# aous72/OpenJPH

Measured on AMD Instinct MI355X. Metric: Msamples/s encode+decode, 8K 12-bit 4:4:4; achieved HBM GB/s vs roofline, higher is better.
Workload: dtype f32; 1 GPU; c3_8k_444_12b_irv97; width=7680, height=4320, components=3, bit_depth=12, wavelet=9/7 irreversible, decomps=5, hip_streams=1, sample_container_bits=16, roundtrip_max_abs_err=8

## Files before the change

include/ojphgpu.h:

```cpp
#ifndef OJPHGPU_H
#define OJPHGPU_H
#include <stddef.h>
#include <stdint.h>

#ifdef __cplusplus
extern "C" {
#endif

#define OJPHGPU_OK              0
#define OJPHGPU_E_INVALID      -1
#define OJPHGPU_E_NOMEM        -2
#define OJPHGPU_E_HIP          -3
#define OJPHGPU_E_CODESTREAM   -4
#define OJPHGPU_E_OVERFLOW     -5
#define OJPHGPU_E_BLOCK        -6
#define OJPHGPU_E_AGAIN        -7
#define OJPHGPU_E_UNCOLLECTED  -8
#define OJPHGPU_E_BUDGET       -9
#define OJPHGPU_E_QUALITY      -10

#define OJPHGPU_MAX_SUBSAMPLED_COMPS 16
#define OJPHGPU_MAX_COC_COMPS 16
#define OJPHGPU_MAX_LIFT_STEPS 16
#define OJPHGPU_MAX_ATK 4
// ... 276 lines not shown
typedef struct ojphgpu_decoder ojphgpu_decoder;

int  ojphgpu_encoder_create(const ojphgpu_plan* plan, int device, void* stream, ojphgpu_encoder** out);
void ojphgpu_encoder_destroy(ojphgpu_encoder* enc);
int  ojphgpu_encoder_create_tiles(const ojphgpu_plan* plan, int device, void* stream,
                                  uint32_t tile_first, uint32_t tile_count, ojphgpu_encoder** out);
int  ojphgpu_encoder_finish_tiles(ojphgpu_encoder* enc, uint8_t* h_out, size_t cap, size_t* out_len,
                                  uint32_t* tile_part_len);
int  ojphgpu_encoder_finish_tiles_device(ojphgpu_encoder* enc, uint8_t* d_out, size_t cap, size_t* out_len,
                                         uint32_t* tile_part_len);
int  ojphgpu_encoder_create_batch(const ojphgpu_plan* plan, int device, void* stream,
                                  uint32_t num_frames, ojphgpu_encoder** out);
int  ojphgpu_encoder_finish_frame(ojphgpu_encoder* enc, uint32_t frame, uint8_t* h_out, size_t cap,
                                  size_t* out_len);
int  ojphgpu_encoder_run_device(ojphgpu_encoder* enc, const int32_t* d_image);
int  ojphgpu_encoder_run_device16(ojphgpu_encoder* enc, const uint16_t* d_image);
int  ojphgpu_encoder_run_device8(ojphgpu_encoder* enc, const uint8_t* d_image);
int  ojphgpu_encode16(ojphgpu_encoder* enc, const uint16_t* h_image, uint8_t* h_out, size_t cap, size_t* out_len);
int  ojphgpu_encoder_finish(ojphgpu_encoder* enc, uint8_t* h_out, size_t cap, size_t* out_len);
int  ojphgpu_encode(ojphgpu_encoder* enc, const int32_t* h_image, uint8_t* h_out, size_t cap,
                    size_t* out_len);
int  ojphgpu_encoder_coded_bytes(ojphgpu_encoder* enc, uint64_t* bytes);

int  ojphgpu_decoder_create(const ojphgpu_plan* plan, int device, void* stream, ojphgpu_decoder** out);
int  ojphgpu_decoder_create_tiles(const ojphgpu_plan* plan, int device, void* stream,
                                  uint32_t tile_first, uint32_t tile_count, ojphgpu_decoder** out);
int  ojphgpu_decoder_create_batch(const ojphgpu_plan* const* plans, uint32_t num_frames, int device,
                                  void* stream, ojphgpu_decoder** out);
int  ojphgpu_decoder_upload_frame(ojphgpu_decoder* dec, uint32_t frame, const uint8_t* h_codestream,
                                  size_t len);
// ... 236 lines not shown
```

openjph_amd/capi.py:

```python
import ctypes as C
import os

_HERE = os.path.dirname(os.path.abspath(__file__))
LIB_PATH = os.path.join(_HERE, "libojphgpu.so")

OK, E_INVALID, E_NOMEM, E_HIP, E_CODESTREAM, E_OVERFLOW, E_BLOCK, E_AGAIN, E_UNCOLLECTED, E_BUDGET, E_QUALITY = 0, -1, -2, -3, -4, -5, -6, -7, -8, -9, -10
RATE_GRID, STATS_BINS = 241, 80
VIDEO_V410, VIDEO_Y410, VIDEO_R210, VIDEO_R10K, VIDEO_Y4XX, VIDEO_AYUV, VIDEO_BGRA, VIDEO_RGBA, VIDEO_ARGB = range(0x21, 0x2A)
PROG_ORDERS = {"LRCP": 0, "RLCP": 1, "RPCL": 2, "PCRL": 3, "CPRL": 4}


class Coc(C.Structure):
    _fields_ = [
        ("rank", C.c_uint8), ("reversible", C.c_uint8), ("num_decomps", C.c_uint8),
        ("log_block_w", C.c_uint8), ("log_block_h", C.c_uint8), ("has_precincts", C.c_uint8),
        ("reserved", C.c_uint8 * 2), ("precinct_exps", C.c_uint8 * 36),
    ]


class LiftStep(C.Structure):
    _fields_ = [("a", C.c_int32), ("b", C.c_int32), ("e", C.c_int32), ("A", C.c_float)]


class Atk(C.Structure):
# ... 269 lines not shown
    "ojphgpu_encoder_destroy": (None, [C.c_void_p]),
    "ojphgpu_encoder_run_device": (C.c_int, [C.c_void_p, C.c_void_p]),
    "ojphgpu_encoder_finish": (C.c_int, [C.c_void_p, C.c_void_p, C.c_size_t, C.POINTER(C.c_size_t)]),
    "ojphgpu_encode": (C.c_int, [C.c_void_p, C.c_void_p, C.c_void_p, C.c_size_t, C.POINTER(C.c_size_t)]),
    "ojphgpu_encoder_coded_bytes": (C.c_int, [C.c_void_p, C.POINTER(C.c_uint64)]),
    "ojphgpu_decoder_create": (C.c_int, [C.c_void_p, C.c_int, C.c_void_p, C.POINTER(C.c_void_p)]),
    "ojphgpu_decoder_destroy": (None, [C.c_void_p]),
    "ojphgpu_decoder_upload": (C.c_int, [C.c_void_p, C.c_void_p, C.c_size_t]),
    "ojphgpu_decoder_run_device": (C.c_int, [C.c_void_p, C.c_void_p]),
    "ojphgpu_decoder_failed_blocks": (C.c_int, [C.c_void_p, C.POINTER(C.c_uint32)]),
    "ojphgpu_decoder_fused_retries": (C.c_int, [C.c_void_p, C.POINTER(C.c_uint32)]),
    "ojphgpu_decoder_giveup_epoch": (C.c_int, [C.c_void_p, C.POINTER(C.c_uint32), C.POINTER(C.c_uint32)]),
    "ojphgpu_decode": (C.c_int, [C.c_void_p, C.c_void_p, C.c_size_t, C.c_void_p]),
    "ojphgpu_encoder_ht_timing": (C.c_int, [C.c_void_p, C.POINTER(C.c_float), C.c_uint32, C.POINTER(C.c_uint32), C.POINTER(C.c_uint32)]),
    "ojphgpu_encoder_set_timing": (C.c_int, [C.c_void_p, C.c_int]),
    "ojphgpu_decoder_set_timing": (C.c_int, [C.c_void_p, C.c_int]),
    "ojphgpu_encoder_timing": (C.c_int, [C.c_void_p, C.POINTER(C.c_float)]),
    "ojphgpu_decoder_timing": (C.c_int, [C.c_void_p, C.POINTER(C.c_float)]),
    "ojphgpu_encoder_level_timing": (C.c_int, [C.c_void_p, C.POINTER(C.c_float), C.c_uint32, C.POINTER(C.c_uint32)]),
    "ojphgpu_decoder_level_timing": (C.c_int, [C.c_void_p, C.POINTER(C.c_float), C.c_uint32, C.POINTER(C.c_uint32)]),
    "ojphgpu_enc_pipe_create": (C.c_int, [C.c_void_p, C.c_int, C.c_uint32, C.c_int, C.c_uint32, C.POINTER(C.c_void_p)]),
    "ojphgpu_enc_pipe_destroy": (None, [C.c_void_p]),
    "ojphgpu_enc_pipe_acquire": (C.c_int, [C.c_void_p, C.POINTER(C.c_void_p), C.POINTER(C.c_size_t)]),
    "ojphgpu_enc_pipe_submit": (C.c_int, [C.c_void_p]),
    "ojphgpu_enc_pipe_collect": (C.c_int, [C.c_void_p, C.POINTER(C.c_void_p), C.POINTER(C.c_size_t)]),
    "ojphgpu_enc_pipe_stats": (C.c_int, [C.c_void_p, C.POINTER(C.c_double)]),
    "ojphgpu_dec_pipe_create": (C.c_int, [C.c_void_p, C.c_size_t, C.c_int, C.c_int, C.c_uint32, C.c_int, C.c_uint32,
                                          C.POINTER(C.c_void_p)]),
    "ojphgpu_dec_pipe_destroy": (None, [C.c_void_p]),
    "ojphgpu_dec_pipe_plan": (C.c_int, [C.c_void_p, C.POINTER(C.c_void_p)]),
# ... 149 lines not shown
```

openjph_amd/codec.py:

```python
import ctypes as C
import numpy as np

from . import capi
from .capi import check, Params, DwtDesc, DwtRegion, CbDesc, CbResult, ConvertDesc
from .plan import Plan, make_params, parse_codestream

dwt_desc_dtype = np.dtype(DwtDesc)
dwt_region_dtype = np.dtype(DwtRegion)
cb_desc_dtype = np.dtype(CbDesc)
cb_result_dtype = np.dtype(CbResult)
convert_desc_dtype = np.dtype(ConvertDesc)


def _torch():
    import torch
    if not torch.cuda.is_available():
        raise RuntimeError("openjph_amd: no GPU visible (torch.cuda.is_available() is False); "
                           "the HTJ2K hot path has no CPU fallback")
    return torch


def _stream_ptr(torch, device):
    return C.c_void_p(torch.cuda.current_stream(device).cuda_stream)

# ... 146 lines not shown
        torch = _torch()
        assert d_image.is_cuda and tuple(d_image.shape) == self.shape and d_image.is_contiguous()
        self._frame = d_image if self.max_sse is not None else None
        if d_image.dtype in (torch.int16, torch.uint16):
            check(self._lib.ojphgpu_encoder_run_device16(self._h, C.c_void_p(d_image.data_ptr())), "encoder_run_device16")
            return
        if d_image.dtype in (torch.int8, torch.uint8):
            check(self._lib.ojphgpu_encoder_run_device8(self._h, C.c_void_p(d_image.data_ptr())), "encoder_run_device8")
            return
        assert d_image.dtype == torch.int32
        check(self._lib.ojphgpu_encoder_run_device(self._h, C.c_void_p(d_image.data_ptr())), "encoder_run_device")

    def set_timing(self, per_launch: bool):
        check(self._lib.ojphgpu_encoder_set_timing(self._h, int(per_launch)), "encoder_set_timing")

    def coded_bytes(self):
        n = C.c_uint64()
        check(self._lib.ojphgpu_encoder_coded_bytes(self._h, C.byref(n)), "encoder_coded_bytes")
        return int(n.value)

    def finish(self, frame=0) -> bytes:
        if self.max_bytes:
            budget = self.budgets[frame] if self.budgets and 0 <= frame < self.frames else self.max_bytes
            cap = min(budget, self.plan.frame_elems * 4 + 64 * self.plan.num_blocks + (1 << 20))
        elif self.max_sse is not None:
            cap = self.plan.frame_elems * 3 + 64 * self.plan.num_blocks + (1 << 20)
        else:
            cap = self.coded_bytes() // self.frames * 2 + 64 * self.plan.num_blocks + (1 << 20)
        out = np.empty(cap, np.uint8)
        n = C.c_size_t()
# ... 771 lines not shown
```

openjph_amd/csrc/ojphgpu_codec.cpp:

```cpp
#include <hip/hip_runtime.h>

#include <algorithm>
#include <chrono>
#include <cstdio>
#include <cstdlib>
#include <cstring>
#include <memory>
#include <mutex>
#include <new>
#include <vector>

#include "ht_tables.h"
#include "ojph_plan.h"
#include "ojph_pool.h"

using namespace ojphgpu;

namespace ojphgpu {

int ensure_tables()
{
  static std::mutex mu;
  static bool done[64] = { false };
  int dev = 0;
// ... 4 lines not shown
  static bool built = false;
  if (!built) { build_ht_tables(tables); built = true; }
  if (upload_enc_tables(tables) != 0 || upload_dec_tables(tables) != 0) return -1;
  done[dev] = true;
  return 0;
}

}

#include "ojphgpu_objects.h"

extern "C" void ojphgpu_encoder_destroy(ojphgpu_encoder* e)
{
  if (!e) return;
  (void)hipSetDevice(e->device);
  for (DeviceBuf* b : { &e->arena, &e->image, &e->dwt_descs, &e->img_descs, &e->cb_descs, &e->conv_descs, &e->scratch, &e->out,
                        &e->results, &e->counters, &e->regions }) b->release();
  e->h_out.release(); e->h_res.release();
  if (e->side) (void)hipStreamDestroy(e->side);
  if (e->ev_fork) (void)hipEventDestroy(e->ev_fork);
  if (e->ev_join) (void)hipEventDestroy(e->ev_join);
  e->timer.destroy();
  delete e->quality;
  delete e->rate;
  delete e;
}

extern "C" int ojphgpu_encoder_create(const ojphgpu_plan* plan, int device, void* stream, ojphgpu_encoder** out)
{
  if (!plan) return OJPHGPU_E_INVALID;
  return ojphgpu_encoder_create_tiles(plan, device, stream, 0, (uint32_t)plan->plan.tiles.size(), out);
}

static int encoder_create(const ojphgpu_plan* plan, int device, void* stream, uint32_t tile_first, uint32_t tile_count,
                          uint32_t nframes, ojphgpu_encoder** out, bool blocks_only = false);

extern "C" int ojphgpu_encoder_create_tiles(const ojphgpu_plan* plan, int device, void* stream, uint32_t tile_first,
                                             uint32_t tile_count, ojphgpu_encoder** out)
{
  return no_throw([&] { return encoder_create(plan, device, stream, tile_first, tile_count, 1, out); });
}

extern "C" int ojphgpu_encoder_create_batch(const ojphgpu_plan* plan, int device, void* stream, uint32_t num_frames,
                                             ojphgpu_encoder** out)
{
  if (!plan) return OJPHGPU_E_INVALID;
  return no_throw([&] { return encoder_create(plan, device, stream, 0, (uint32_t)plan->plan.tiles.size(), num_frames, out); });
}

static void encoder_block_layout(ojphgpu_encoder* e, const uint32_t* band_kmax, std::vector<ojphgpu_cb_desc>& bd, uint64_t& scratch_total,
                                 bool* clamped = nullptr)
{
  if (clamped) *clamped = false;
  const Plan& P = *e->P;
  const uint32_t nframes = e->nframes;
// ... 51 lines not shown
        if (clamped) *clamped = true;
        R = 0; break;
      }
      e->h_regions[2 * r] = (uint32_t)total; e->h_regions[2 * r + 1] = (uint32_t)c;
      total += c;
    }
    e->nreg = R;
    if (R) cap = total; else e->h_regions.clear();
    e->counters_bytes = R ? (size_t)R * 128 : 16;
  }
  e->out_cap = (uint32_t)cap;
  scratch_total = scratch_bytes;
}

static int encoder_create(const ojphgpu_plan* plan, int device, void* stream, uint32_t tile_first, uint32_t tile_count,
                          uint32_t nframes, ojphgpu_encoder** out, bool blocks_only)
{
  if (!plan || !out || nframes == 0) return OJPHGPU_E_INVALID;
  *out = nullptr;
  if ((uint64_t)tile_first + tile_count > plan->plan.tiles.size()) return OJPHGPU_E_INVALID;
  if (plan->plan.skip_read || plan->plan.skip_recon) return OJPHGPU_E_INVALID;
  HIPCHK(hipSetDevice(device));
  if (ensure_tables() != 0) return OJPHGPU_E_HIP;
  ojphgpu_encoder* e = new (std::nothrow) ojphgpu_encoder();
  if (!e) return OJPHGPU_E_NOMEM;
  struct Owner { ojphgpu_encoder* p; ~Owner() { if (p) ojphgpu_encoder_destroy(p); } } owner{ e };
  const Plan& P = plan->plan;
  e->handle = plan; e->P = &P; e->device = device; e->stream = (hipStream_t)stream;
  auto bail = [&](int rc) { return rc; };

  e->tiles = TileRange{ tile_first, tile_count };
// ... 14 lines not shown
    auto top = [&](uint32_t id) { const Band& B = P.bands[P.blocks[id].band]; return B.res == P.style(B.comp).L; };
    auto mid = std::stable_partition(e->block_ids.begin(), e->block_ids.end(), top);
    e->n_top = (uint32_t)(mid - e->block_ids.begin());
    {
      static const int share_env = [] { const char* v = getenv("OJPHGPU_ENC_TOP_SHARE"); const int x = v ? atoi(v) : 0; return x < 10 ? 0 : x > 100 ? 100 : x; }();
      double s_top = 0, s_low = 0;
      for (size_t i = 0; i < e->block_ids.size(); ++i) {
        const Block& k = P.blocks[e->block_ids[i]];
        (i < e->n_top ? s_top : s_low) += (double)k.r.w * k.r.h * 1e-6;
      }
      double dwt_us = 0, level_bytes = 8.0 * (s_top + s_low) * 1e6 / 4.0;
      for (uint32_t l = 2; l <= max_recon_decomps(P); ++l, level_bytes /= 4.0) dwt_us += std::max(12.0, level_bytes / 3.0e6);
      const double us_per_ms = 3.8, margin_us = 30.0;
      const double move = (s_top + margin_us / us_per_ms - 1.6 * s_low - dwt_us / us_per_ms) / 2.0;
      int share = share_env;
      if (!share) share = s_top > 0 && move > 0 ? (int)(100.0 * (1.0 - move / s_top)) : 100;
      share = share < 50 ? 50 : share > 100 ? 100 : share;
      e->n_top = (uint32_t)((uint64_t)e->n_top * (uint32_t)share / 100u);
    }
    if (e->n_top == 0 || e->n_top == e->block_ids.size()) e->n_top = 0;
    else {
      int prio_lo = 0, prio_hi = 0;
      (void)hipDeviceGetStreamPriorityRange(&prio_lo, &prio_hi);
      const char* pe = getenv("OJPHGPU_ENC_SIDE_PRIO");
      const int prio = pe && pe[0] == 'l' ? prio_lo : pe && pe[0] == 'h' ? prio_hi : (prio_lo + prio_hi) / 2;
      if (hipStreamCreateWithPriority(&e->side, hipStreamNonBlocking, pe ? prio : 0) != hipSuccess ||
          hipEventCreateWithFlags(&e->ev_fork, hipEventDisableTiming) != hipSuccess ||
          hipEventCreateWithFlags(&e->ev_join, hipEventDisableTiming) != hipSuccess) return bail(OJPHGPU_E_HIP);
    }
  }
  std::vector<ojphgpu_cb_desc> bd;
  uint64_t scratch_bytes = 0;
  encoder_block_layout(e, nullptr, bd, scratch_bytes);
  const uint64_t cap = e->out_cap;

  if ((!blocks_only && (e->arena.alloc(P.arena_elems * 4 * nframes) || e->dwt_descs.alloc(dd.size() * sizeof(dd[0])) ||
                        e->img_descs.alloc(idd.size() * sizeof(dd[0])) || e->conv_descs.alloc(cd.size() * sizeof(cd[0])))) ||
      e->cb_descs.alloc(bd.size() * sizeof(bd[0])) ||
      e->scratch.alloc(scratch_bytes) || e->out.alloc(cap) ||
      e->results.alloc(bd.size() * sizeof(ojphgpu_cb_result)) || e->counters.alloc(e->counters_bytes) ||
      (e->nreg && e->regions.alloc(e->h_regions.size() * 4)))
    return bail(OJPHGPU_E_NOMEM);
  if (e->nreg && hipMemcpy(e->regions.p, e->h_regions.data(), e->h_regions.size() * 4, hipMemcpyHostToDevice) != hipSuccess) return bail(OJPHGPU_E_HIP);
// ... 15 lines not shown
extern "C" int ojphgpu_encoder_run_device16(ojphgpu_encoder* e, const uint16_t* d_image) { return ojphgpu_encoder_run_container(e, d_image, 16); }
extern "C" int ojphgpu_encoder_run_device8(ojphgpu_encoder* e, const uint8_t* d_image) { return ojphgpu_encoder_run_container(e, d_image, 8); }

namespace {
struct BlockCoderRun {
  ojphgpu_encoder* e; uint8_t* out; ojphgpu_cb_result* res; uint32_t* cnt; uint32_t nblocks; Spans* T;
  bool forked = false;
  int launch(hipStream_t st, uint32_t first, uint32_t n, int widths) {
    const int sh = T ? T->begin(SP_HT_ENC, st) : -1;
    int rc = ojphgpu::ht_encode_launch(st, (const ojphgpu_cb_desc*)e->cb_descs.p + first, n, e->arena.p, (uint8_t*)e->scratch.p, out,
                                       e->out_cap, res + first, cnt, cnt + 1, widths, (const uint32_t*)e->regions.p, e->nreg);
    if (rc) return rc;
    if (T) T->end(sh, st);
    return OJPHGPU_OK;
  }
  int clear() { HIPCHK(hipMemsetAsync(cnt, 0, e->counters_bytes, e->stream)); return OJPHGPU_OK; }
  int fork_top() {
    forked = true;
    HIPCHK(hipEventRecord(e->ev_fork, e->stream));
    HIPCHK(hipStreamWaitEvent(e->side, e->ev_fork, 0));
    int rc = launch(e->side, 0, e->n_top, e->widths_top);
    if (rc) return rc;
    HIPCHK(hipEventRecord(e->ev_join, e->side));
    return OJPHGPU_OK;
  }
  int rest_and_join() {
    int rc = e->n_top && !forked ? fork_top() : OJPHGPU_OK;
    if (rc) return rc;
    rc = launch(e->stream, e->n_top, nblocks - e->n_top, e->widths_rest);
    if (rc) return rc;
    if (e->n_top) HIPCHK(hipStreamWaitEvent(e->stream, e->ev_join, 0));
    return OJPHGPU_OK;
  }
};
}

int ojphgpu_encoder_run_container(ojphgpu_encoder* e, const void* d_image, int container)
{
  if (!e || !d_image) return OJPHGPU_E_INVALID;
  const Plan& P = *e->P;
  if (container != 32 && container != 16 && container != 8) return OJPHGPU_E_INVALID;
  if (container != 32) for (const CompGeo& g : P.comps) if (g.bit_depth > (uint32_t)container) return OJPHGPU_E_INVALID;
  hipStream_t s = e->stream;
  Spans& T = e->timer;
  BlockCoderRun coder{ e, (uint8_t*)(e->o_out ? e->o_out : e->out.p),
                       (ojphgpu_cb_result*)(e->o_results ? e->o_results : e->results.p),
                       (uint32_t*)(e->o_counters ? e->o_counters : e->counters.p), (uint32_t)e->block_ids.size() * e->nframes, &T };
  int rc = coder.clear();
  if (rc) return rc;
  T.start(s);
  if (e->need_convert) {
    const int sp = T.begin(SP_CONVERT, s);
    rc = ojphgpu_convert_forward_ex(s, &P.p, (const ojphgpu_convert_desc*)e->conv_descs.p, e->tiles.count * e->nframes,
                                    e->conv_max_w, e->conv_max_h, d_image, e->arena.p, container);
    T.end(sp, s);
  }
  if (rc) return rc;
  const bool budget = e->searches();
  for (size_t i = 0; i < e->batches.size(); ++i) {
    const LevelBatch& b = e->batches[i];
    const int sp = T.begin(SP_DWT, s);
    if (b.img_first >= 0) {
      ojphgpu_params pp = P.p; pp.reversible = b.rev ? 1 : 0; pp.bit_depth = b.img_depth; pp.is_signed = b.img_signed;
      const ojphgpu_dwt_desc* idesc = (const ojphgpu_dwt_desc*)e->img_descs.p + b.img_first;
      rc = b.general ? ojphgpu_dwt_forward_general_image(s, &b.k, &pp, idesc, b.count, b.max_w, b.max_h, d_image, e->arena.p, container)
                     : ojphgpu_dwt_forward_image_ex(s, &pp, idesc, b.count, b.max_w, b.max_h, d_image, e->arena.p, container, b.nc == 3);
    } else if (b.general)
      rc = ojphgpu_dwt_forward_general(s, &b.k, (const ojphgpu_dwt_desc*)e->dwt_descs.p + b.first, b.count, b.max_w, b.max_h, e->arena.p);
    else
      rc = ojphgpu_dwt_forward(s, b.rev ? 1 : 0, (const ojphgpu_dwt_desc*)e->dwt_descs.p + b.first, b.count,
                               b.max_w, b.max_h, e->arena.p);
    if (rc) return rc;
    T.end(sp, s);
    const bool top_done = b.depth == 0 && (i + 1 == e->batches.size() || e->batches[i + 1].depth != 0);
    if (!budget && e->n_top && top_done && (rc = coder.fork_top()) != 0) return rc;
  }
  if (e->quality_on) {
    T.finish(s);
    e->quality->frame = d_image; e->quality->container = container;
    e->rate->searched = false;
    e->ran = true; e->fetched = false;
    return OJPHGPU_OK;
  }
  if (budget) {
    EncoderRate& R = *e->rate;
    HIPCHK(hipMemsetAsync(R.hist.p, 0, R.hist.n, s));
    const int sp = T.begin(SP_STATS, s);
    rc = ojphgpu_band_stats(s, (const ojphgpu_stats_desc*)R.stats_descs.p, R.n_stats, R.stats_max_w, R.stats_max_h, e->arena.p, (uint32_t*)R.hist.p);
    if (rc) return rc;
    T.end(sp, s);
    T.finish(s);
    R.searched = false;
    e->ran = true; e->fetched = false;
    return OJPHGPU_OK;
  }
  if ((rc = coder.rest_and_join()) != 0) return rc;
  T.finish(s);
  e->ran = true; e->fetched = false;
  return OJPHGPU_OK;
}

extern "C" int ojphgpu_encoder_set_timing(ojphgpu_encoder* e, int per_launch)
{
  if (!e) return OJPHGPU_E_INVALID;
  e->timer.detail = per_launch != 0;
  return OJPHGPU_OK;
}

extern "C" int ojphgpu_encoder_coded_bytes(ojphgpu_encoder* e, uint64_t* bytes)
{
  if (!e || !bytes || !e->ran) return OJPHGPU_E_INVALID;
  e->h_cursors.assign(e->counters_bytes / 4, 0);
  HIPCHK(hipMemcpyAsync(e->h_cursors.data(), e->counters.p, e->counters_bytes, hipMemcpyDeviceToHost, e->stream));
  HIPCHK(hipStreamSynchronize(e->stream));
  uint64_t total = e->h_cursors[0];
  for (uint32_t r = 1; r < e->nreg; ++r) total += e->h_cursors[32 * (size_t)r];
  *bytes = total;
  return e->h_cursors[1] ? OJPHGPU_E_OVERFLOW : OJPHGPU_OK;
}

static int encoder_fetch(ojphgpu_encoder* e, uint32_t frame, std::vector<ojphgpu_coded_block>& cb)
{
  if (frame >= e->nframes) return OJPHGPU_E_INVALID;
  const Plan& P = e->searches() ? e->rate->frame_plan[frame]->plan : *e->P;
  if (!e->fetched) {
    int rc = ojphgpu_encoder_coded_bytes(e, &e->nbytes);
// ... 108 lines not shown
    if (lay.alloc(boff + L.blob.size() + 64)) return OJPHGPU_E_NOMEM;
    struct Free { DeviceBuf& b; ~Free() { b.release(); } } fr{ lay };
    if (jbytes) HIPCHK(hipMemcpyAsync(lay.p, L.jobs.data(), jbytes, hipMemcpyHostToDevice, e->stream));
    if (!L.blob.empty()) HIPCHK(hipMemcpyAsync((uint8_t*)lay.p + boff, L.blob.data(), L.blob.size(), hipMemcpyHostToDevice, e->stream));
    rc = assemble_launch(e->stream, (const T2Job*)lay.p, (uint32_t)L.jobs.size(), (const uint8_t*)lay.p + boff,
                         (const uint8_t*)(e->o_out ? e->o_out : e->out.p), d_out);
    if (rc) return rc;
    HIPCHK(hipStreamSynchronize(e->stream));
    return OJPHGPU_OK;
  });
}

static int encoder_restore_descs(ojphgpu_encoder* e)
{
  HIPCHK(hipSetDevice(e->device));
  HIPCHK(hipStreamSynchronize(e->stream));
  const std::vector<ojphgpu_cb_desc>& bd = e->rate->bd;
  if (!bd.empty()) HIPCHK(hipMemcpy(e->cb_descs.p, bd.data(), bd.size() * sizeof(bd[0]), hipMemcpyHostToDevice));
  e->ran = false;
  return OJPHGPU_OK;
}

static bool encoder_may_search(const ojphgpu_encoder* e)
{
  const Plan& P = *e->P;
  return e->tiles.first == 0 && e->tiles.count == P.tiles.size() && !e->o_out && rate_plan_ok(P);
}

static int encoder_rate_setup(ojphgpu_encoder* e);

// ... 51 lines not shown
    const uint32_t nc = R->table.nclasses;
    std::vector<uint32_t> kfine(P.bands.size());
    for (size_t i = 0; i < kfine.size(); ++i) kfine[i] = R->table.quant[(size_t)(OJPHGPU_RATE_GRID - 1) * nc + R->table.band_class[i]].K_max;
    std::vector<ojphgpu_cb_desc>& bd = R->bd;
    uint64_t scratch_bytes = 0;
    {
      const uint32_t out_cap = e->out_cap, nreg = e->nreg; const size_t counters_bytes = e->counters_bytes;
      const std::vector<uint32_t> regions = e->h_regions;
      bool clamped = false;
      encoder_block_layout(e, kfine.data(), bd, scratch_bytes, &clamped);
      if (clamped && nframes > 1) {
        e->out_cap = out_cap; e->nreg = nreg; e->counters_bytes = counters_bytes; e->h_regions = regions;
        return OJPHGPU_E_INVALID;
      }
    }
    HIPCHK(hipStreamSynchronize(e->stream));
    if (e->side) HIPCHK(hipStreamSynchronize(e->side));
    e->scratch.release(); e->out.release(); e->regions.release(); e->counters.release();
    if (e->scratch.alloc(scratch_bytes) || e->out.alloc(e->out_cap) || e->counters.alloc(e->counters_bytes) ||
        (e->nreg && e->regions.alloc(e->h_regions.size() * 4)) ||
        R->stats_descs.alloc(sd.size() * sizeof(sd[0])) || R->hist.alloc(P.bands.size() * OJPHGPU_STATS_BINS * 4 * nframes) ||
        R->block_class.alloc(cls.size() * 4) || R->quant.alloc((size_t)nc * sizeof(BandQuant) * nframes))
      return OJPHGPU_E_NOMEM;
    if (e->nreg) HIPCHK(hipMemcpy(e->regions.p, e->h_regions.data(), e->h_regions.size() * 4, hipMemcpyHostToDevice));
    if (!bd.empty()) HIPCHK(hipMemcpy(e->cb_descs.p, bd.data(), bd.size() * sizeof(bd[0]), hipMemcpyHostToDevice));
    if (!sd.empty()) HIPCHK(hipMemcpy(R->stats_descs.p, sd.data(), sd.size() * sizeof(sd[0]), hipMemcpyHostToDevice));
    if (!cls.empty()) HIPCHK(hipMemcpy(R->block_class.p, cls.data(), cls.size() * 4, hipMemcpyHostToDevice));
    R->h_hist.assign(P.bands.size() * OJPHGPU_STATS_BINS * nframes, 0);
    R->h_quant.assign((size_t)nc * nframes, BandQuant{ 0.0f, 0 });
    e->rate = R; owner.p = nullptr;
// ... 373 lines not shown
}

extern "C" int ojphgpu_encode(ojphgpu_encoder* e, const int32_t* h_image, uint8_t* h_out, size_t cap, size_t* out_len)
{
  return encode_host(e, h_image, 32, h_out, cap, out_len);
}

extern "C" int ojphgpu_encode16(ojphgpu_encoder* e, const uint16_t* h_image, uint8_t* h_out, size_t cap, size_t* out_len)
{
  return encode_host(e, h_image, 16, h_out, cap, out_len);
}

extern "C" int ojphgpu_encoder_timing(ojphgpu_encoder* e, float out[4])
{
  if (!e || !out || !e->ran) return OJPHGPU_E_INVALID;
  if (e->timer.read(SP_CONVERT, &out[0]) || e->timer.read(SP_DWT, &out[1]) || e->timer.read(SP_HT_ENC, &out[2]) ||
      e->timer.read(-1, &out[3])) return OJPHGPU_E_HIP;
  return OJPHGPU_OK;
}

extern "C" int ojphgpu_encoder_ht_timing(ojphgpu_encoder* e, float* out, uint32_t cap, uint32_t* n, uint32_t* n_top)
{
  if (!e || !out || !n || !e->ran) return OJPHGPU_E_INVALID;
  int k = e->timer.read_each(SP_HT_ENC, out, cap);
  if (k < 0) return OJPHGPU_E_HIP;
  *n = (uint32_t)k;
  if (n_top) *n_top = e->n_top;
  return OJPHGPU_OK;
}

extern "C" int ojphgpu_encoder_level_timing(ojphgpu_encoder* e, float* out, uint32_t cap, uint32_t* n)
{
  if (!e || !out || !n || !e->ran) return OJPHGPU_E_INVALID;
  int k = e->timer.read_each(SP_DWT, out, cap);
  if (k < 0) return OJPHGPU_E_HIP;
  *n = (uint32_t)k;
  return OJPHGPU_OK;
}

extern "C" void ojphgpu_decoder_destroy(ojphgpu_decoder* d)
{
  if (!d) return;
  (void)hipSetDevice(d->device);
  for (DeviceBuf* b : { &d->arena, &d->image, &d->dwt_descs, &d->img_descs, &d->cb_descs, &d->conv_descs, &d->data, &d->status, &d->quads, &d->aux,
                       &d->fstate, &d->dwt_regs, &d->img_regs })
    b->release();
  if (d->h_retry) (void)hipHostFree(d->h_retry);
  if (d->h_stage) (void)hipHostFree(d->h_stage);
// ... 887 lines not shown
```

openjph_amd/csrc/ojphgpu_objects.h:

```cpp
#ifndef OJPHGPU_OBJECTS_H
#define OJPHGPU_OBJECTS_H
#include <hip/hip_runtime.h>

#include <algorithm>
#include <cstdint>
#include <cstdlib>
#include <cstring>
#include <map>
#include <vector>

#include "dwt_region.h"
#include "ht_tables.h"
#include "ojph_plan.h"

using namespace ojphgpu;

namespace {

#define HIPCHK(x) do { if ((x) != hipSuccess) return OJPHGPU_E_HIP; } while (0)

struct DeviceBuf {
  void* p = nullptr; size_t n = 0;
  int alloc(size_t bytes) { n = bytes; return hipMalloc(&p, bytes ? bytes : 16) == hipSuccess ? 0 : -1; }
  void release() { if (p) (void)hipFree(p); p = nullptr; }
// ... 317 lines not shown
std::vector<uint32_t> blocks_of_tiles(const Plan& P, TileRange tr)
{
  std::vector<uint32_t> ids;
  for (size_t i = 0; i < P.blocks.size(); ++i) {
    const Band& B = P.bands[P.blocks[i].band];
    if (P.has_region && !P.reg_blocks[i]) continue;
    if (tr.has(B.tile) && B.res <= P.top_read_res(B.comp)) ids.push_back((uint32_t)i);
  }
  return ids;
}

struct Spans {
  struct Span { hipEvent_t a, b; int kind; };
  std::vector<Span> pool;
  size_t used = 0;
  hipEvent_t t0 = nullptr, t1 = nullptr;
  bool ok = false;
  bool detail = true;
  int init() { ok = hipEventCreate(&t0) == hipSuccess && hipEventCreate(&t1) == hipSuccess; return ok ? 0 : -1; }
  void destroy() {
    for (Span& x : pool) { (void)hipEventDestroy(x.a); (void)hipEventDestroy(x.b); }
    if (t0) (void)hipEventDestroy(t0);
    if (t1) (void)hipEventDestroy(t1);
    pool.clear();
  }
  void start(hipStream_t s) { used = 0; if (ok) (void)hipEventRecord(t0, s); }
  void finish(hipStream_t s) { if (ok) (void)hipEventRecord(t1, s); }
  int begin(int kind, hipStream_t s) {
    if (!ok || !detail) return -1;
    if (used == pool.size()) {
      Span x{ nullptr, nullptr, kind };
      if (hipEventCreate(&x.a) != hipSuccess || hipEventCreate(&x.b) != hipSuccess) { ok = false; return -1; }
      pool.push_back(x);
    }
    pool[used].kind = kind;
    (void)hipEventRecord(pool[used].a, s);
    return (int)used++;
  }
  void end(int id, hipStream_t s) { if (ok && id >= 0) (void)hipEventRecord(pool[(size_t)id].b, s); }
  int read(int kind, float* out) {
    if (!ok || hipEventSynchronize(t1) != hipSuccess) return -1;
    if (kind < 0) return hipEventElapsedTime(out, t0, t1) == hipSuccess ? 0 : -1;
    float sum = 0;
    for (size_t i = 0; i < used; ++i)
      if (pool[i].kind == kind) { float ms = 0; if (hipEventElapsedTime(&ms, pool[i].a, pool[i].b) != hipSuccess) return -1; sum += ms; }
    *out = sum;
    return 0;
  }
  int read_each(int kind, float* out, uint32_t cap) {
    if (!ok || hipEventSynchronize(t1) != hipSuccess) return -1;
    int n = 0;
    for (size_t i = 0; i < used; ++i)
      if (pool[i].kind == kind && (uint32_t)n < cap) { if (hipEventElapsedTime(&out[n], pool[i].a, pool[i].b) != hipSuccess) return -1; ++n; }
    return n;
  }
};
enum { SP_CONVERT = 0, SP_DWT = 1, SP_HT_ENC = 2, SP_PREP = 3, SP_STEP1 = 4, SP_STEP2 = 5, SP_REFINE = 6, SP_STATS = 7 };
// ... 48 lines not shown
  std::vector<LevelBatch> batches;
  uint32_t conv_max_w = 0, conv_max_h = 0, out_cap = 0;
  TileRange tiles{ 0, 0 };
  uint32_t nframes = 1;
  bool fetched = false;
  uint64_t nbytes = 0;
  std::vector<uint32_t> block_ids;
  std::vector<ojphgpu_cb_result> h_results;
  HostBuf h_out, h_res;
  Spans timer;
  bool ran = false;
  uint32_t n_top = 0;
  int widths_top = 0, widths_rest = 0;
  hipStream_t side = nullptr;
  hipEvent_t ev_fork = nullptr, ev_join = nullptr;
  void* o_out = nullptr; void* o_results = nullptr; void* o_counters = nullptr;
  uint32_t nreg = 0;
  std::vector<uint32_t> h_regions, h_cursors;
  DeviceBuf regions;
  size_t counters_bytes = 16;
  std::vector<uint64_t> budgets;
  EncoderRate* rate = nullptr;
  bool quality_on = false; uint64_t max_sse = 0;
  uint64_t cap_bytes = 0;
  EncoderQuality* quality = nullptr;
  bool searches() const { return !budgets.empty() || quality_on; }
};
struct RateTrialOut {
  void* out; ojphgpu_cb_result* d_results; uint32_t* d_counters;
  const ojphgpu_cb_result* h_results; uint32_t* d_publish; const uint32_t* h_publish; hipEvent_t done;
};
int64_t ojphgpu_encoder_rate_trial(ojphgpu_encoder* e, Plan& Q, const RateTrialOut& o, uint32_t j);
struct QualityTrialIo {
  const void* frame; int container;
  ojphgpu_requant_desc* h_descs; const void* d_descs;
  const ojphgpu_frame_err* h_err; void* d_err; hipEvent_t done;
};
int ojphgpu_encoder_quality_trial(ojphgpu_encoder* e, const QualityTrialIo& io, uint32_t j, ojphgpu_frame_err* comps);
int ojphgpu_encoder_run_container(ojphgpu_encoder* e, const void* d_image, int container);

inline void ojphgpu_coded_blocks(const Plan& P, const std::vector<uint32_t>& block_ids, const ojphgpu_cb_result* res,
                                 std::vector<ojphgpu_coded_block>& cb)
{
  cb.assign(P.blocks.size(), ojphgpu_coded_block{ 0, 0, 0, 0, 0 });
  for (size_t i = 0; i < block_ids.size(); ++i) {
    const ojphgpu_cb_result& r = res[i];
    ojphgpu_coded_block& c = cb[block_ids[i]];
    c.offset = r.offset; c.len1 = r.length; c.len2 = 0;
    c.missing_msbs = r.length ? P.bands[P.blocks[block_ids[i]].band].K_max - 1 : 0;
    c.num_passes = r.length ? 1 : 0;
  }
}

struct PadCopy { uint64_t src, dst; uint32_t got, total; };
// ... 84 lines not shown
```

openjph_amd/csrc/ojphgpu_pipe.cpp:

```cpp
#include <chrono>
#include <condition_variable>
#include <deque>
#include <mutex>
#include <new>
#include <thread>

#include "ojphgpu_objects.h"
#include "ojph_pool.h"
#include "video_formats.h"

namespace ojphgpu {
int assemble_launch(void* stream, const T2Job* d_jobs, uint32_t njobs, const uint8_t* d_blob, const uint8_t* d_data, uint8_t* d_out);
int copy_to_host_launch(void* stream, void* d_dst, const void* src, size_t bytes);
int publish_words_launch(void* stream, uint32_t* d_dst, const uint32_t* src, uint32_t n);
int gather_runs_launch(void* stream, const void* d_src, size_t src_cap, const void* d_runs, uint32_t nruns, void* d_dst, uint64_t staged_len);
}

namespace {

struct Pinned {
  uint8_t* p = nullptr; uint8_t* d = nullptr; size_t cap = 0;
  int reserve(size_t bytes) {
    if (bytes <= cap) return 0;
    release();
// ... 499 lines not shown
extern "C" int ojphgpu_enc_pipe_create(const ojphgpu_plan* plan, int device, uint32_t depth, int container_bits,
                                        uint32_t host_threads, ojphgpu_enc_pipe** out)
{
  if (!plan || !out || depth < 2 || depth > 16 || (container_bits != 8 && container_bits != 16 && container_bits != 32)) return OJPHGPU_E_INVALID;
  *out = nullptr;
  return no_throw([&]() -> int {
    HIPCHK(hipSetDevice(device));
    ojphgpu_enc_pipe* p = new (std::nothrow) ojphgpu_enc_pipe();
    if (!p) return OJPHGPU_E_NOMEM;
    struct Owner { ojphgpu_enc_pipe* p; ~Owner() { if (p) ojphgpu_enc_pipe_destroy(p); } } owner{ p };
    const Plan& P = plan->plan;
    p->handle = plan; p->P = &P; p->device = device; p->container = container_bits; p->depth = depth;
    if (container_bits != 32) for (const CompGeo& g : P.comps) if (g.bit_depth > (uint32_t)container_bits) return OJPHGPU_E_INVALID;
    for (hipStream_t* s : { &p->s_h2d, &p->s_comp }) HIPCHK(hipStreamCreateWithFlags(s, hipStreamNonBlocking));
    HIPCHK(create_copy_out_stream(&p->s_d2h));
    int rc = ojphgpu_encoder_create(plan, device, p->s_comp, &p->enc);
    if (rc) return rc;
    (void)ojphgpu_encoder_set_timing(p->enc, 0);
    ojphgpu_encoder* e = p->enc;
    const size_t nb = e->block_ids.size();
    p->frame_bytes = (size_t)P.frame_elems * (size_t)(container_bits / 8);
    p->ho.bytes = p->frame_bytes;
    p->res_bytes = nb * sizeof(ojphgpu_cb_result) + 16;
    const size_t cs_guess = std::min<size_t>((size_t)e->out_cap, (size_t)P.frame_elems + (1u << 20));
    p->slots.resize(depth);
    for (EncSlot& s : p->slots) {
      if (s.h_in.reserve(p->frame_bytes + 64) || s.o.h_res.reserve(p->res_bytes + 64) || s.h_cs.reserve(cs_guess)) return OJPHGPU_E_NOMEM;
      if (s.image.alloc(p->frame_bytes + 64) || s.o.out.alloc((size_t)e->out_cap + 64) || s.o.counters.alloc(e->counters_bytes) ||
          s.cs.reserve(cs_guess)) return OJPHGPU_E_NOMEM;
      const size_t lay_guess = nb * sizeof(T2Job) + nb * 8 + (1u << 16);
      if (s.h_lay.reserve(lay_guess)) return OJPHGPU_E_NOMEM;
// ... 945 lines not shown
```

Before: 107,800 Msamples/s.

## Release encoder's HT block coding onto low-priority streams without joining main stream

When the encoder forks the top-level HT block coding onto a side stream, the remaining blocks now go onto a second low-priority stream instead of the main stream. Neither branch is joined back to the main stream; the encoder is marked pending and every later consumer (clear, coded_bytes, timing, restore, destroy) first settles by making the main stream wait on both branch events. This aims to let the tail of HT encoding overlap with subsequent work such as the decode or the next frame. The cost is extra synchronisation bookkeeping and a risk of missed settle points, so the pipe encoder opts out by using a joined-only constructor.

```diff
diff --git a/include/ojphgpu.h b/include/ojphgpu.h
--- a/include/ojphgpu.h
+++ b/include/ojphgpu.h
@@ -314,6 +314,7 @@
 int  ojphgpu_encoder_finish_frame(ojphgpu_encoder* enc, uint32_t frame, uint8_t* h_out, size_t cap,
                                   size_t* out_len);
 int  ojphgpu_encoder_run_device(ojphgpu_encoder* enc, const int32_t* d_image);
+int  ojphgpu_encoder_is_pending(const ojphgpu_encoder* enc, int* pending);
 int  ojphgpu_encoder_run_device16(ojphgpu_encoder* enc, const uint16_t* d_image);
 int  ojphgpu_encoder_run_device8(ojphgpu_encoder* enc, const uint8_t* d_image);
 int  ojphgpu_encode16(ojphgpu_encoder* enc, const uint16_t* h_image, uint8_t* h_out, size_t cap, size_t* out_len);
diff --git a/openjph_amd/capi.py b/openjph_amd/capi.py
--- a/openjph_amd/capi.py
+++ b/openjph_amd/capi.py
@@ -307,6 +307,7 @@
     "ojphgpu_decode": (C.c_int, [C.c_void_p, C.c_void_p, C.c_size_t, C.c_void_p]),
     "ojphgpu_encoder_ht_timing": (C.c_int, [C.c_void_p, C.POINTER(C.c_float), C.c_uint32, C.POINTER(C.c_uint32), C.POINTER(C.c_uint32)]),
     "ojphgpu_encoder_set_timing": (C.c_int, [C.c_void_p, C.c_int]),
+    "ojphgpu_encoder_is_pending": (C.c_int, [C.c_void_p, C.POINTER(C.c_int)]),
     "ojphgpu_decoder_set_timing": (C.c_int, [C.c_void_p, C.c_int]),
     "ojphgpu_encoder_timing": (C.c_int, [C.c_void_p, C.POINTER(C.c_float)]),
     "ojphgpu_decoder_timing": (C.c_int, [C.c_void_p, C.POINTER(C.c_float)]),
diff --git a/openjph_amd/codec.py b/openjph_amd/codec.py
--- a/openjph_amd/codec.py
+++ b/openjph_amd/codec.py
@@ -184,6 +184,11 @@
     def set_timing(self, per_launch: bool):
         check(self._lib.ojphgpu_encoder_set_timing(self._h, int(per_launch)), "encoder_set_timing")
 
+    def pending(self):
+        n = C.c_int()
+        check(self._lib.ojphgpu_encoder_is_pending(self._h, C.byref(n)), "encoder_is_pending")
+        return bool(n.value)
+
     def coded_bytes(self):
         n = C.c_uint64()
         check(self._lib.ojphgpu_encoder_coded_bytes(self._h, C.byref(n)), "encoder_coded_bytes")
diff --git a/openjph_amd/csrc/ojphgpu_codec.cpp b/openjph_amd/csrc/ojphgpu_codec.cpp
--- a/openjph_amd/csrc/ojphgpu_codec.cpp
+++ b/openjph_amd/csrc/ojphgpu_codec.cpp
@@ -42,12 +42,17 @@
 {
   if (!e) return;
   (void)hipSetDevice(e->device);
+  if (e->side) (void)hipStreamSynchronize(e->side);
+  if (e->low) (void)hipStreamSynchronize(e->low);
+  e->pending = false;
   for (DeviceBuf* b : { &e->arena, &e->image, &e->dwt_descs, &e->img_descs, &e->cb_descs, &e->conv_descs, &e->scratch, &e->out,
                         &e->results, &e->counters, &e->regions }) b->release();
   e->h_out.release(); e->h_res.release();
   if (e->side) (void)hipStreamDestroy(e->side);
+  if (e->low) (void)hipStreamDestroy(e->low);
   if (e->ev_fork) (void)hipEventDestroy(e->ev_fork);
   if (e->ev_join) (void)hipEventDestroy(e->ev_join);
+  if (e->ev_low) (void)hipEventDestroy(e->ev_low);
   e->timer.destroy();
   delete e->quality;
   delete e->rate;
@@ -61,12 +66,18 @@
 }
 
 static int encoder_create(const ojphgpu_plan* plan, int device, void* stream, uint32_t tile_first, uint32_t tile_count,
-                          uint32_t nframes, ojphgpu_encoder** out, bool blocks_only = false);
+                          uint32_t nframes, ojphgpu_encoder** out, bool blocks_only = false, bool joined_only = false);
 
 extern "C" int ojphgpu_encoder_create_tiles(const ojphgpu_plan* plan, int device, void* stream, uint32_t tile_first,
                                              uint32_t tile_count, ojphgpu_encoder** out)
 {
   return no_throw([&] { return encoder_create(plan, device, stream, tile_first, tile_count, 1, out); });
+}
+
+int ojphgpu_encoder_create_joined(const ojphgpu_plan* plan, int device, void* stream, ojphgpu_encoder** out)
+{
+  if (!plan) return OJPHGPU_E_INVALID;
+  return no_throw([&] { return encoder_create(plan, device, stream, 0, (uint32_t)plan->plan.tiles.size(), 1, out, false, true); });
 }
 
 extern "C" int ojphgpu_encoder_create_batch(const ojphgpu_plan* plan, int device, void* stream, uint32_t num_frames,
@@ -148,7 +159,7 @@
 }
 
 static int encoder_create(const ojphgpu_plan* plan, int device, void* stream, uint32_t tile_first, uint32_t tile_count,
-                          uint32_t nframes, ojphgpu_encoder** out, bool blocks_only)
+                          uint32_t nframes, ojphgpu_encoder** out, bool blocks_only, bool joined_only)
 {
   if (!plan || !out || nframes == 0) return OJPHGPU_E_INVALID;
   *out = nullptr;
@@ -193,8 +204,7 @@
       const double us_per_ms = 3.8, margin_us = 30.0;
       const double move = (s_top + margin_us / us_per_ms - 1.6 * s_low - dwt_us / us_per_ms) / 2.0;
       int share = share_env;
-      if (!share) share = s_top > 0 && move > 0 ? (int)(100.0 * (1.0 - move / s_top)) : 100;
-      share = share < 50 ? 50 : share > 100 ? 100 : share;
+      if (!share) { share = s_top > 0 && move > 0 ? (int)(100.0 * (1.0 - move / s_top)) : 100; share = share < 50 ? 50 : share > 100 ? 100 : share; }
       e->n_top = (uint32_t)((uint64_t)e->n_top * (uint32_t)share / 100u);
     }
     if (e->n_top == 0 || e->n_top == e->block_ids.size()) e->n_top = 0;
@@ -203,9 +213,15 @@
       (void)hipDeviceGetStreamPriorityRange(&prio_lo, &prio_hi);
       const char* pe = getenv("OJPHGPU_ENC_SIDE_PRIO");
       const int prio = pe && pe[0] == 'l' ? prio_lo : pe && pe[0] == 'h' ? prio_hi : (prio_lo + prio_hi) / 2;
-      if (hipStreamCreateWithPriority(&e->side, hipStreamNonBlocking, pe ? prio : 0) != hipSuccess ||
+      const char* rel = getenv("OJPHGPU_ENC_RELEASE");
+      e->can_release = !blocks_only && !joined_only && !(rel && rel[0] == '0');
+      const int own_prio = pe ? prio : e->can_release ? prio_lo : 0;
+      if (hipStreamCreateWithPriority(&e->side, hipStreamNonBlocking, own_prio) != hipSuccess ||
           hipEventCreateWithFlags(&e->ev_fork, hipEventDisableTiming) != hipSuccess ||
           hipEventCreateWithFlags(&e->ev_join, hipEventDisableTiming) != hipSuccess) return bail(OJPHGPU_E_HIP);
+      if (e->can_release &&
+          (hipStreamCreateWithPriority(&e->low, hipStreamNonBlocking, own_prio) != hipSuccess ||
+           hipEventCreateWithFlags(&e->ev_low, hipEventDisableTiming) != hipSuccess)) return bail(OJPHGPU_E_HIP);
     }
   }
   std::vector<ojphgpu_cb_desc> bd;
@@ -251,16 +267,18 @@
     if (T) T->end(sh, st);
     return OJPHGPU_OK;
   }
-  int clear() { HIPCHK(hipMemsetAsync(cnt, 0, e->counters_bytes, e->stream)); return OJPHGPU_OK; }
-  int fork_top() {
+  int clear() { int rc = encoder_settle(e); if (rc) return rc; HIPCHK(hipMemsetAsync(cnt, 0, e->counters_bytes, e->stream)); return OJPHGPU_OK; }
+  int fork_top(bool release = false) {
     forked = true;
     HIPCHK(hipEventRecord(e->ev_fork, e->stream));
     HIPCHK(hipStreamWaitEvent(e->side, e->ev_fork, 0));
     int rc = launch(e->side, 0, e->n_top, e->widths_top);
     if (rc) return rc;
     HIPCHK(hipEventRecord(e->ev_join, e->side));
+    if (release) { e->pending = true; HIPCHK(hipStreamWaitEvent(e->low, e->ev_fork, 0)); }
     return OJPHGPU_OK;
   }
+  int rest_released() { return launch(e->low, e->n_top, nblocks - e->n_top, e->widths_rest); }
   int rest_and_join() {
     int rc = e->n_top && !forked ? fork_top() : OJPHGPU_OK;
     if (rc) return rc;
@@ -269,6 +287,10 @@
     if (e->n_top) HIPCHK(hipStreamWaitEvent(e->stream, e->ev_join, 0));
     return OJPHGPU_OK;
   }
+};
+struct ReleasedBranch {
+  ojphgpu_encoder* e; bool armed = false;
+  ~ReleasedBranch() { if (armed) (void)hipEventRecord(e->ev_low, e->low); }
 };
 }
 
@@ -285,6 +307,8 @@
                        (uint32_t*)(e->o_counters ? e->o_counters : e->counters.p), (uint32_t)e->block_ids.size() * e->nframes, &T };
   int rc = coder.clear();
   if (rc) return rc;
+  const bool release = encoder_releases(e);
+  ReleasedBranch branch{ e };
   T.start(s);
   if (e->need_convert) {
     const int sp = T.begin(SP_CONVERT, s);
@@ -310,7 +334,10 @@
     if (rc) return rc;
     T.end(sp, s);
     const bool top_done = b.depth == 0 && (i + 1 == e->batches.size() || e->batches[i + 1].depth != 0);
-    if (!budget && e->n_top && top_done && (rc = coder.fork_top()) != 0) return rc;
+    if (!budget && e->n_top && top_done) {
+      if ((rc = coder.fork_top(release)) != 0) return rc;
+      if (release) { s = e->low; branch.armed = true; }
+    }
   }
   if (e->quality_on) {
     T.finish(s);
@@ -331,8 +358,13 @@
     e->ran = true; e->fetched = false;
     return OJPHGPU_OK;
   }
-  if ((rc = coder.rest_and_join()) != 0) return rc;
-  T.finish(s);
+  if (release && coder.forked) {
+    if ((rc = coder.rest_released()) != 0) return rc;
+    T.finish_two(s, e->side);
+  } else {
+    if ((rc = coder.rest_and_join()) != 0) return rc;
+    T.finish(s);
+  }
   e->ran = true; e->fetched = false;
   return OJPHGPU_OK;
 }
@@ -344,9 +376,18 @@
   return OJPHGPU_OK;
 }
 
+extern "C" int ojphgpu_encoder_is_pending(const ojphgpu_encoder* e, int* pending)
+{
+  if (!e || !pending) return OJPHGPU_E_INVALID;
+  *pending = e->pending ? 1 : 0;
+  return OJPHGPU_OK;
+}
+
 extern "C" int ojphgpu_encoder_coded_bytes(ojphgpu_encoder* e, uint64_t* bytes)
 {
   if (!e || !bytes || !e->ran) return OJPHGPU_E_INVALID;
+  int rc = encoder_settle(e);
+  if (rc) return rc;
   e->h_cursors.assign(e->counters_bytes / 4, 0);
   HIPCHK(hipMemcpyAsync(e->h_cursors.data(), e->counters.p, e->counters_bytes, hipMemcpyDeviceToHost, e->stream));
   HIPCHK(hipStreamSynchronize(e->stream));
@@ -485,6 +526,8 @@
 static int encoder_restore_descs(ojphgpu_encoder* e)
 {
   HIPCHK(hipSetDevice(e->device));
+  int rc = encoder_settle(e);
+  if (rc) return rc;
   HIPCHK(hipStreamSynchronize(e->stream));
   const std::vector<ojphgpu_cb_desc>& bd = e->rate->bd;
   if (!bd.empty()) HIPCHK(hipMemcpy(e->cb_descs.p, bd.data(), bd.size() * sizeof(bd[0]), hipMemcpyHostToDevice));
@@ -566,6 +609,7 @@
         return OJPHGPU_E_INVALID;
       }
     }
+    { const int rc = encoder_settle(e); if (rc) return rc; }
     HIPCHK(hipStreamSynchronize(e->stream));
     if (e->side) HIPCHK(hipStreamSynchronize(e->side));
     e->scratch.release(); e->out.release(); e->regions.release(); e->counters.release();
@@ -969,6 +1013,7 @@
 extern "C" int ojphgpu_encoder_timing(ojphgpu_encoder* e, float out[4])
 {
   if (!e || !out || !e->ran) return OJPHGPU_E_INVALID;
+  if (encoder_settle(e)) return OJPHGPU_E_HIP;
   if (e->timer.read(SP_CONVERT, &out[0]) || e->timer.read(SP_DWT, &out[1]) || e->timer.read(SP_HT_ENC, &out[2]) ||
       e->timer.read(-1, &out[3])) return OJPHGPU_E_HIP;
   return OJPHGPU_OK;
@@ -977,6 +1022,7 @@
 extern "C" int ojphgpu_encoder_ht_timing(ojphgpu_encoder* e, float* out, uint32_t cap, uint32_t* n, uint32_t* n_top)
 {
   if (!e || !out || !n || !e->ran) return OJPHGPU_E_INVALID;
+  if (encoder_settle(e)) return OJPHGPU_E_HIP;
   int k = e->timer.read_each(SP_HT_ENC, out, cap);
   if (k < 0) return OJPHGPU_E_HIP;
   *n = (uint32_t)k;
@@ -987,6 +1033,7 @@
 extern "C" int ojphgpu_encoder_level_timing(ojphgpu_encoder* e, float* out, uint32_t cap, uint32_t* n)
 {
   if (!e || !out || !n || !e->ran) return OJPHGPU_E_INVALID;
+  if (encoder_settle(e)) return OJPHGPU_E_HIP;
   int k = e->timer.read_each(SP_DWT, out, cap);
   if (k < 0) return OJPHGPU_E_HIP;
   *n = (uint32_t)k;
diff --git a/openjph_amd/csrc/ojphgpu_objects.h b/openjph_amd/csrc/ojphgpu_objects.h
--- a/openjph_amd/csrc/ojphgpu_objects.h
+++ b/openjph_amd/csrc/ojphgpu_objects.h
@@ -355,18 +355,21 @@
   struct Span { hipEvent_t a, b; int kind; };
   std::vector<Span> pool;
   size_t used = 0;
-  hipEvent_t t0 = nullptr, t1 = nullptr;
+  hipEvent_t t0 = nullptr, t1 = nullptr, t2 = nullptr;
   bool ok = false;
   bool detail = true;
-  int init() { ok = hipEventCreate(&t0) == hipSuccess && hipEventCreate(&t1) == hipSuccess; return ok ? 0 : -1; }
+  bool two = false;
+  int init() { ok = hipEventCreate(&t0) == hipSuccess && hipEventCreate(&t1) == hipSuccess && hipEventCreate(&t2) == hipSuccess; return ok ? 0 : -1; }
   void destroy() {
     for (Span& x : pool) { (void)hipEventDestroy(x.a); (void)hipEventDestroy(x.b); }
     if (t0) (void)hipEventDestroy(t0);
     if (t1) (void)hipEventDestroy(t1);
+    if (t2) (void)hipEventDestroy(t2);
     pool.clear();
   }
-  void start(hipStream_t s) { used = 0; if (ok) (void)hipEventRecord(t0, s); }
+  void start(hipStream_t s) { used = 0; two = false; if (ok) (void)hipEventRecord(t0, s); }
   void finish(hipStream_t s) { if (ok) (void)hipEventRecord(t1, s); }
+  void finish_two(hipStream_t s, hipStream_t other) { finish(s); two = ok; if (ok) (void)hipEventRecord(t2, other); }
   int begin(int kind, hipStream_t s) {
     if (!ok || !detail) return -1;
     if (used == pool.size()) {
@@ -381,7 +384,13 @@
   void end(int id, hipStream_t s) { if (ok && id >= 0) (void)hipEventRecord(pool[(size_t)id].b, s); }
   int read(int kind, float* out) {
     if (!ok || hipEventSynchronize(t1) != hipSuccess) return -1;
-    if (kind < 0) return hipEventElapsedTime(out, t0, t1) == hipSuccess ? 0 : -1;
+    if (kind < 0) {
+      if (hipEventElapsedTime(out, t0, t1) != hipSuccess) return -1;
+      float other = 0;
+      if (two && (hipEventSynchronize(t2) != hipSuccess || hipEventElapsedTime(&other, t0, t2) != hipSuccess)) return -1;
+      *out = std::max(*out, other);
+      return 0;
+    }
     float sum = 0;
     for (size_t i = 0; i < used; ++i)
       if (pool[i].kind == kind) { float ms = 0; if (hipEventElapsedTime(&ms, pool[i].a, pool[i].b) != hipSuccess) return -1; sum += ms; }
@@ -460,6 +469,9 @@
   int widths_top = 0, widths_rest = 0;
   hipStream_t side = nullptr;
   hipEvent_t ev_fork = nullptr, ev_join = nullptr;
+  hipStream_t low = nullptr;
+  hipEvent_t ev_low = nullptr;
+  bool pending = false, can_release = false;
   void* o_out = nullptr; void* o_results = nullptr; void* o_counters = nullptr;
   uint32_t nreg = 0;
   std::vector<uint32_t> h_regions, h_cursors;
@@ -472,6 +484,18 @@
   EncoderQuality* quality = nullptr;
   bool searches() const { return !budgets.empty() || quality_on; }
 };
+inline bool encoder_releases(const ojphgpu_encoder* e)
+{
+  return e->can_release && e->n_top && !e->o_out && !e->o_results && !e->o_counters && !e->searches() && !e->timer.detail;
+}
+inline int encoder_settle(ojphgpu_encoder* e)
+{
+  if (!e->pending) return OJPHGPU_OK;
+  HIPCHK(hipStreamWaitEvent(e->stream, e->ev_join, 0));
+  HIPCHK(hipStreamWaitEvent(e->stream, e->ev_low, 0));
+  e->pending = false;
+  return OJPHGPU_OK;
+}
 struct RateTrialOut {
   void* out; ojphgpu_cb_result* d_results; uint32_t* d_counters;
   const ojphgpu_cb_result* h_results; uint32_t* d_publish; const uint32_t* h_publish; hipEvent_t done;
@@ -484,6 +508,7 @@
 };
 int ojphgpu_encoder_quality_trial(ojphgpu_encoder* e, const QualityTrialIo& io, uint32_t j, ojphgpu_frame_err* comps);
 int ojphgpu_encoder_run_container(ojphgpu_encoder* e, const void* d_image, int container);
+int ojphgpu_encoder_create_joined(const ojphgpu_plan* plan, int device, void* stream, ojphgpu_encoder** out);
 
 inline void ojphgpu_coded_blocks(const Plan& P, const std::vector<uint32_t>& block_ids, const ojphgpu_cb_result* res,
                                  std::vector<ojphgpu_coded_block>& cb)
diff --git a/openjph_amd/csrc/ojphgpu_pipe.cpp b/openjph_amd/csrc/ojphgpu_pipe.cpp
--- a/openjph_amd/csrc/ojphgpu_pipe.cpp
+++ b/openjph_amd/csrc/ojphgpu_pipe.cpp
@@ -537,7 +537,7 @@
     if (container_bits != 32) for (const CompGeo& g : P.comps) if (g.bit_depth > (uint32_t)container_bits) return OJPHGPU_E_INVALID;
     for (hipStream_t* s : { &p->s_h2d, &p->s_comp }) HIPCHK(hipStreamCreateWithFlags(s, hipStreamNonBlocking));
     HIPCHK(create_copy_out_stream(&p->s_d2h));
-    int rc = ojphgpu_encoder_create(plan, device, p->s_comp, &p->enc);
+    int rc = ojphgpu_encoder_create_joined(plan, device, p->s_comp, &p->enc);
     if (rc) return rc;
     (void)ojphgpu_encoder_set_timing(p->enc, 0);
     ojphgpu_encoder* e = p->enc;
```

Measured after the change: 110,200 Msamples/s, median of 6. 2.2% higher.
